# consilience-dev/llm-map-reduce-summarizer

Measured on AMD Instinct MI355X. Metric: chunks/sec (whole node) + end-to-end wall-clock, 10h transcript, Llama-3-8B, higher is better.
Workload: dtype bf16

## Files before the change

llm_map_reduce_summarizer_amd/csrc/kernels/stream_gemm.hip:

```cpp
#include "ar_common.h"

namespace {
enum { EPI_BF16 = 0, EPI_F32_PARTIAL = 1, EPI_SWIGLU = 2, EPI_SWIGLU_SPLIT = 3, EPI_RESID_SPLIT = 4 };
constexpr int SS_PARTS = 8;
constexpr int KBLK = 128;
constexpr int LDS_XTRA = 3 * 1024;
constexpr int LDS_BUDGET = 160 * 1024 - LDS_XTRA;

struct NormArgs {
    const float* ssq;
    int ssq_tiles;
    float inv_k, eps;
    bf16* resid;
    int ldr;
    float* ssp;
    int slab_m;
    mrsum_ar::TPPush tp;
};

template <int N>
__device__ __forceinline__ void wait_vmcnt() {
    static_assert(N >= 0 && N < 64, "vmcnt range");
    __builtin_amdgcn_s_waitcnt((N & 15) | (7 << 4) | (15 << 8) | ((N >> 4) << 14));
}
// ... 756 lines not shown
    }
#pragma unroll
    for (int o = 32; o > 0; o >>= 1) m = max(m, (uint32_t)__shfl_xor((int)m, o, 64));
    if ((threadIdx.x & 63) == 0) atomicMax(stats, (int)m);
}

__global__ __launch_bounds__(64) void p14_pack_kernel(const bf16* __restrict__ W, int K, unsigned char* __restrict__ P,
                                                      int* __restrict__ stats) {
    const int lane = threadIdx.x, r = lane & 15, g = lane >> 4;
    const int nkb = K / KBLK;
    const size_t tile = blockIdx.x;
    const int G = (int)(tile / nkb), kb = (int)(tile % nkb);
    const int base7 = max(stats[0] - 30, 1);
    const uint4* src = reinterpret_cast<const uint4*>(W + (size_t)(16 * G + r) * K + (size_t)kb * KBLK + 8 * g);
    uint32_t lo[8], nb[4], s2[2] = {0u, 0u};
    int bad = 0;
#pragma unroll
    for (int i = 0; i < 4; ++i) {
        const uint4 v = src[4 * i];
        const uint32_t d[4] = {v.x, v.y, v.z, v.w};
        lo[2 * i] = lo[2 * i + 1] = nb[i] = 0u;
#pragma unroll
        for (int el = 0; el < 8; ++el) {
            const uint32_t wv = (d[el >> 1] >> (16 * (el & 1))) & 0xffffu;
            const int e7 = (wv >> 8) & 0x7f, c = e7 ? e7 - base7 + 1 : 0;
            bad += e7 && (c < 1 || c > 31);
            const uint32_t c5 = (uint32_t)c & 31u, sg = wv >> 15;
            const int b = el & 3, q = 2 * (i & 1) + (el >> 2);
            lo[2 * i + (el >> 2)] |= (wv & 0xffu) << (8 * b);
            nb[i] |= (c5 & 15u) << (8 * b + 4 * (el >> 2));
            s2[i >> 1] |= (c5 >> 4) << (8 * b + 4 - q) | sg << (8 * b + 7 - (q == 3 ? 7 : q));
        }
    }
    unsigned char* t = P + tile * P14_TILE;
    *reinterpret_cast<uint4*>(t + 16 * lane) = make_uint4(lo[0], lo[1], lo[2], lo[3]);
    *reinterpret_cast<uint4*>(t + 1024 + 16 * lane) = make_uint4(lo[4], lo[5], lo[6], lo[7]);
    *reinterpret_cast<uint4*>(t + P14_NIB + 16 * lane) = make_uint4(nb[0], nb[1], nb[2], nb[3]);
    *reinterpret_cast<uint2*>(t + P14_TWO + 8 * lane) = make_uint2(s2[0], s2[1]);
    if (bad) atomicAdd(stats + 1, bad);
}
}

MRSUM_API int mrsum_p14_pack(const void* W, int N, int K, void* packed, int* stats, hipStream_t s) {
    if (N <= 0 || K <= 0 || N % 16 || K % KBLK || !W || !packed || !stats) return (int)hipErrorInvalidValue;
    hipError_t rc = hipMemsetAsync(stats, 0, 2 * sizeof(int), s);
    if (rc != hipSuccess) return (int)rc;
    const size_t n16 = (size_t)N * K / 8;
    const int blocks = (int)((n16 + 255) / 256 < 4096 ? (n16 + 255) / 256 : 4096);
    p14_max_kernel<<<blocks, 256, 0, s>>>((const uint4*)W, n16, stats);
    p14_pack_kernel<<<(unsigned)((size_t)(N / 16) * (K / KBLK)), 64, 0, s>>>((const bf16*)W, K, (unsigned char*)packed,
                                                                              stats);
    return (int)hipGetLastError();
}
```

llm_map_reduce_summarizer_amd/engine/model.py:

```python

from __future__ import annotations

import hashlib
import math
import os
from dataclasses import dataclass
from typing import Callable, List, Optional

import torch

from .. import ops
from ..ops.reference import Fp8Weight, interleave_gate_up, rope_cos_sin
from ..parallel.dist import AsyncWorks
from .config import ModelConfig


def _seed_for(seed: int, name: str) -> int:
    return int.from_bytes(hashlib.sha1(("%d:%s" % (seed, name)).encode()).digest()[:8], "little") & ((1 << 63) - 1)


def _randn(shape, std: float, seed: int, name: str, device, dtype) -> torch.Tensor:
    g = torch.Generator(device=device)
    g.manual_seed(_seed_for(seed, name))
    t = torch.randn(*shape, generator=g, device=device, dtype=torch.float32 if device.type == "cpu" else dtype)
    t.mul_(std)
    return t.to(dtype)


class _TPReduce:

    def __init__(self, model: "LlamaModel"):
        self.model = model
        ar = model.custom_ar
        self.fused = ar is not None and os.environ.get("MRSUM_FUSED_AR", "1") == "1"

    def __call__(self, t: torch.Tensor) -> torch.Tensor:
        return self.model._all_reduce(t)

    def fused_ok(self, rows: int, hidden: int) -> bool:
        ar = self.model.custom_ar
        return self.fused and ar is not None and ar.paths["fused_norm"] and rows <= ar.MAX_ROWS and \
            hidden % 4 == 0 and hidden <= 8192 and rows * hidden * 2 <= ar.max_bytes

    def add_rmsnorm(self, parts, residual, ln, eps):
        return self.model.custom_ar.add_rmsnorm(parts, residual, ln, eps)

    def push_ok(self, rows: int, hidden: int) -> bool:
        ar = self.model.custom_ar
        return ar is not None and _tp_push_enabled() and ar.push_ok(rows, hidden)

    def push_handle(self) -> int:
        return self.model.custom_ar.push_handle()

    def push_kinds(self) -> set:
        return self.model.custom_ar.push_kinds()


def _page_of(kcache: torch.Tensor, head_dim: int) -> int:
# ... 84 lines not shown
                hidden=cfg.hidden, k={"o": self.hq * self.hd, "down": self.ffn_local},
                fp8=weight_dtype == "fp8", rows=(1, 16, 64)))

    def _init_weights(self, seed: int) -> None:
        c, dev, dt = self.cfg, self.device, self.dtype
        std = c.init_std
        r, tp, hd = self.tp_rank, self.tp_size, c.head_dim
        ones = lambda: torch.ones(c.hidden, device=dev, dtype=dt)
        self.embed = _randn((c.vocab_size, c.hidden), std, seed, "embed", dev, dt)
        self.layers: List[LayerWeights] = []
        for i in range(c.n_layers):
            wq = _randn((c.n_heads * hd, c.hidden), std, seed, "l%d.wq" % i, dev, dt)
            wk = _randn((c.n_kv_heads * hd, c.hidden), std, seed, "l%d.wk" % i, dev, dt)
            wv = _randn((c.n_kv_heads * hd, c.hidden), std, seed, "l%d.wv" % i, dev, dt)
            qs, ks = self.hq * hd, self.hkv * hd
            wqkv = torch.cat([wq[r * qs:(r + 1) * qs], wk[r * ks:(r + 1) * ks], wv[r * ks:(r + 1) * ks]]).contiguous()
            del wq, wk, wv
            wo = _randn((c.hidden, c.n_heads * hd), std, seed, "l%d.wo" % i, dev, dt)
            wo = wo[:, r * qs:(r + 1) * qs].contiguous()
            f = self.ffn_local
            wg = _randn((c.ffn, c.hidden), std, seed, "l%d.wg" % i, dev, dt)
            wu = _randn((c.ffn, c.hidden), std, seed, "l%d.wu" % i, dev, dt)
            wgu = interleave_gate_up(wg[r * f:(r + 1) * f], wu[r * f:(r + 1) * f]).contiguous()
            del wg, wu
            wd = _randn((c.hidden, c.ffn), std, seed, "l%d.wd" % i, dev, dt)
            wd = wd[:, r * f:(r + 1) * f].contiguous()
            if self.weight_dtype == "fp8":
                wqkv, wo, wgu, wd = (Fp8Weight.quantize(t) for t in (wqkv, wo, wgu, wd))
            self.layers.append(LayerWeights(ones(), wqkv, wo, ones(), wgu, wd))
        self.final_norm = ones()
        lm = _randn((c.vocab_size, c.hidden), std, seed, "lm_head", dev, dt)
        v = self.vocab_local
        self.lm_head = lm[r * v:(r + 1) * v].contiguous()
        del lm
        self._quantize_lm_head()

    def _quantize_lm_head(self) -> None:
        if self.weight_dtype == "fp8" and not isinstance(self.lm_head, Fp8Weight):
            self.lm_head = Fp8Weight.quantize(self.lm_head)

    def _pack_p14(self) -> None:
        self.p14 = []
        if self.weight_dtype != "bf16" or self.tp_size != 1 or self.device.type != "cuda" \
                or self.dtype != torch.bfloat16:
            return
        hip = _hip()
        if not hip.p14_enabled():
            return
        todo = [(self.lm_head, "lm_head")]
        for lw in self.layers:
            todo += [(lw.wqkv, "qkv"), (lw.wo, "o"), (lw.wgu, "gate_up"), (lw.wdown, "down")]
        for w, role in todo:
            if hip.p14_role_used(role) and w.shape[0] % 16 == 0 and w.shape[1] % 128 == 0:
                self.p14.append(hip.p14_attach(w, role))

    def __del__(self):
        try:
            for pw in getattr(self, "p14", ()):
                _hip().p14_detach(pw.w)
        except Exception:
            pass

    def weight_bytes(self) -> int:
        def nb(t):
            return t.nbytes() if isinstance(t, Fp8Weight) else t.numel() * t.element_size()
        n = nb(self.embed) + nb(self.lm_head) + nb(self.final_norm) + sum(pw.nbytes() for pw in self.p14)
        for lw in self.layers:
            n += sum(nb(t) for t in (lw.ln1, lw.wqkv, lw.wo, lw.ln2, lw.wgu, lw.wdown))
        return n

    def local_push(self):
        if self._local_push is None:
            from ..parallel.custom_ar import LocalPush
            self._local_push = LocalPush()
        return self._local_push

    def _all_reduce(self, t: torch.Tensor) -> torch.Tensor:
        if self.tp_size > 1:
            if self.custom_ar is not None and self.custom_ar.fits(t):
                self.custom_ar.all_reduce(t)
            else:
                if t.is_cuda and torch.cuda.is_current_stream_capturing():
                    raise RuntimeError("TP all-reduce of %s does not fit the P2P buffers inside a hipGraph "
                                       "capture (lower the decode batch or raise max_bytes)" % (tuple(t.shape),))
                torch.distributed.all_reduce(t, group=self.tp_group)
        return t

    def _all_reduce_async(self, t: torch.Tensor):
        if self.tp_size == 1:
            return None
        if self.custom_ar is not None and self.custom_ar.fits(t):
            self.custom_ar.all_reduce(t)
            return None
        return torch.distributed.all_reduce(t, group=self.tp_group, async_op=True)

    def _sp_backend_ok(self) -> bool:
        return True

    def _sp_host(self) -> bool:
        return self.device.type == "cuda" and torch.distributed.get_backend(self.tp_group) != "nccl"

    def _sp_rows(self, T: int):
        Tp = -(-T // self.tp_size) * self.tp_size
        return Tp, Tp // self.tp_size

    def _sp_shard(self, t: torch.Tensor) -> torch.Tensor:
        T = t.shape[0]
# ... 203 lines not shown
```

llm_map_reduce_summarizer_amd/ops/hip.py:

```python

from __future__ import annotations

import ctypes
import os
from typing import Optional

import torch

from ._lib import kernels_lib
from .reference import Fp8Weight

_c_int, _c_float, _vp = ctypes.c_int, ctypes.c_float, ctypes.c_void_p

_SIGS = {
    "mrsum_rmsnorm": [_vp, _vp, _vp, _c_int, _c_int, _c_int, _c_int, _c_float, _vp],
    "mrsum_add_rmsnorm": [_vp, _vp, _vp, _vp, _c_int, _c_int, _c_int, _c_int, _c_float, _vp],
    "mrsum_rmsnorm_fp8": [_vp, _vp, _vp, _vp, _vp, _c_int, _c_int, _c_int, _c_int, _c_float, _c_int, _vp],
    "mrsum_rope_kv": [_vp, _c_int, _c_int, _vp, _vp, _vp, _c_int, _vp, _vp, _vp, _c_int, _c_int, _c_int, _c_int,
                      _c_int, _c_int, _vp],
    "mrsum_rope_kv_parts": [_vp, _c_int, _vp, _c_int, _c_int, _vp, _vp, _vp, _c_int, _vp, _vp, _vp, _c_int,
                            _c_int, _c_int, _c_int, _c_int, _vp],
    "mrsum_swiglu": [_vp, _vp, _c_int, _c_int, _vp],
    "mrsum_kv_scatter": [_vp, _c_int, _c_int, _c_int, _vp, _vp, _vp, _vp, _c_int, _vp],
    "mrsum_embed": [_vp, _vp, _vp, _c_int, _c_int, _c_int, _vp],
    "mrsum_attn_prefill": [_vp, _c_int, _vp, _vp, _c_int, _c_int, _vp, _c_int, _c_int, _c_int, _c_int, _c_float, _vp],
    "mrsum_attn_prefill_paged": [_vp, _c_int, _vp, _vp, _c_int, _c_int, _vp, _c_int, _c_int, _c_int, _c_int, _c_float,
                                 _vp,
                                 _vp, _vp, _c_int, _vp, _vp, _c_int, _vp],
    "mrsum_attn_decode_mfma": [_vp, _c_int, _vp, _vp, _vp, _c_int, _vp, _vp, _vp, _vp, _c_int, _c_int, _c_int,
                               _c_int, _c_int, _c_int, _c_int, _c_float, _vp, _c_int, _vp],
    "mrsum_attn_decode_rope": [_vp, _c_int, _vp, _vp, _vp, _vp, _c_int, _vp, _vp, _vp, _vp, _c_int, _c_int,
                               _c_int, _c_int, _c_int, _c_int, _c_int, _c_float, _vp, _c_int, _vp],
    "mrsum_skinny_gemm": [_vp, _c_int, _vp, _c_int, _c_int, _c_int, _vp, _c_int, _c_int, _c_int, _c_int, _vp, _c_int,
                          _c_float, _vp, _c_int, _vp, _vp, _c_int, _vp],
    "mrsum_skinny_resid_capacity_w": [_c_int],
    "mrsum_skinny_lds": [_vp, _c_int, _vp, _c_int, _c_int, _c_int, _vp, _c_int, _c_int, _c_int, _c_int, _vp],
    "mrsum_stream_gemm": [_vp, _c_int, _vp, _c_int, _c_int, _c_int, _vp, _c_int, _c_int, _c_int, _c_int, _vp, _vp,
                          _vp, _c_int, _c_float, _vp, _c_int, _vp, _c_int, _vp, _vp],
    "mrsum_stream_fp8": [_vp, _c_int, _vp, _vp, _c_int, _c_int, _c_int, _vp, _c_int, _c_int, _c_int, _c_int, _vp, _vp,
                         _vp, _c_int, _c_float, _vp, _c_int, _vp, _vp, _vp],
    "mrsum_stream_p14": [_vp, _c_int, _vp, _c_int, _c_int, _c_int, _c_int, _vp, _c_int, _c_int, _c_int, _c_int, _vp,
                         _vp, _vp, _c_int, _c_float, _vp, _c_int, _vp, _vp, _vp],
    "mrsum_p14_pack": [_vp, _c_int, _c_int, _vp, _vp, _vp],
    "mrsum_skinny_fp8": [_vp, _c_int, _vp, _vp, _c_int, _c_int, _c_int, _vp, _c_int, _c_int, _c_int, _c_int, _vp,
                         _c_int, _c_float, _vp, _c_int, _vp, _vp, _c_int, _vp],
    "mrsum_skinny_fp8_resid_capacity": [],
    "mrsum_quant_fp8_rows": [_vp, _c_int, _vp, _vp, _c_int, _c_int, _vp],
    "mrsum_add_rmsnorm_parts": [_vp, _c_int, _vp, _vp, _vp, _c_int, _c_int, _c_int, _c_float, _vp],
    "mrsum_sample_keys": [_vp, _c_int, _c_int, _c_int, _c_int, _vp, _vp, _vp, _vp, _vp],
    "mrsum_sample_finish": [_vp, _vp, _vp, _vp, _vp, _vp, _c_int, _vp, _vp, _c_int, _vp],
    "mrsum_gemm": [_vp, _c_int, _vp, _c_int, _vp, _c_int, _c_int, _c_int, _c_int, _c_int, _c_int, _vp, _vp, _c_int,
                   _c_int, _vp],
    "mrsum_sample": [_vp, _c_int, _c_int, _c_int, _vp, _vp, _vp, _vp, _vp, _vp, _vp, _vp, _vp, _c_int, _vp, _vp,
                     _vp],
    "mrsum_penalize": [_vp, _c_int, _c_int, _c_int, _c_int, _vp, _c_int, _vp, _vp, _vp, _vp, _vp, _vp],
    "mrsum_penalize_scan": [_vp, _c_int, _c_int, _c_int, _c_int, _vp, _c_int, _vp, _vp, _vp, _vp, _vp, _vp],
    "mrsum_constrain": [_vp, _c_int, _c_int, _c_int, _c_int, _vp, _vp, _c_int, _vp, _vp, _vp, _vp, _vp, _vp, _vp],
    "mrsum_sample_finish_stops": [_vp, _vp, _vp, _vp, _vp, _vp, _c_int, _vp, _vp, _vp, _c_int, _vp],
    "mrsum_sample_keys_filtered": [_vp, _c_int, _c_int, _c_int, _vp, _vp, _vp, _vp, _vp, _vp, _vp, _vp, _vp, _vp],
    "mrsum_sample_thresh": [_vp, _c_int, _c_int, _c_int, _vp, _vp, _vp, _vp, _vp, _vp, _vp],
    "mrsum_sample_filtered": [_vp, _c_int, _c_int, _c_int, _vp, _vp, _vp, _vp, _vp, _vp, _vp, _vp, _vp, _vp, _vp,
                              _vp, _vp, _c_int, _vp, _vp, _vp],
}

_fns = {}


def _fn(name: str):
    f = _fns.get(name)
    if f is None:
        lib = kernels_lib()
        f = getattr(lib, name)
        f.argtypes = _SIGS[name]
        f.restype = ctypes.c_int
        _fns[name] = f
    return f


def _stream() -> int:
    return torch.cuda.current_stream().cuda_stream


def _p(t: Optional[torch.Tensor]) -> Optional[int]:
    return None if t is None else t.data_ptr()


DEBUG_SYNC = os.environ.get("MRSUM_DEBUG_SYNC", "0") == "1"


def _check(rc: int, name: str) -> None:
    if rc != 0:
        raise RuntimeError("%s launch failed: hipError %d" % (name, rc))
    if DEBUG_SYNC and not torch.cuda.is_current_stream_capturing():
        try:
            torch.cuda.synchronize()
        except RuntimeError as e:
# ... 709 lines not shown
    N = w.shape[0]
    if M > SKINNY_MAX_M and epi in (EPI_BF16, EPI_F32_PARTIAL, EPI_SWIGLU) and norm is None:
        ch = STREAM_TALL_M
        for r0 in range(0, M, ch):
            r1 = min(M, r0 + ch)
            if r1 - r0 > SKINNY_MAX_M:
                tw = tall_wpb(N, r1 - r0, splits)
                if tw is not None:
                    o = out[:, r0:r1] if epi == EPI_F32_PARTIAL else out[r0:r1]
                    _stream_launch(x[r0:r1], w, o, epi, splits, ldo, tw, None, None, None, None, None,
                                   M if epi == EPI_F32_PARTIAL else 0)
                    continue
            for c0 in range(r0, r1, SKINNY_MAX_M):
                c1 = min(r1, c0 + SKINNY_MAX_M)
                o = out[:, c0:c1] if epi == EPI_F32_PARTIAL else out[c0:c1]
                _stream_launch(x[c0:c1], w, o, epi, splits, ldo, wpb, None, None, None, None, None,
                               M if epi == EPI_F32_PARTIAL else 0)
        return out
    return _stream_launch(x, w, out, epi, splits, ldo, wpb, parts, counters, norm, resid, ssp, 0, ar)


STREAM_TALL_M = 128
_TALL_WPB = {6: (4, 5, 6), 8: (4, 5)}


def tall_wpb(N: int, M: int, splits: int) -> Optional[int]:
    mt = 6 if M <= 96 else 8
    best, key = None, None
    for wpb in _TALL_WPB[mt]:
        if N % (16 * wpb):
            continue
        grid = N // (16 * wpb) * splits
        k = (round(grid / (-(-grid // N_CU) * N_CU), 3), wpb)
        if key is None or k > key:
            best, key = wpb, k
    return best


def _stream_launch(x, w, out, epi, splits, ldo, wpb, parts, counters, norm, resid, ssp, slab_m, ar=None):
    M, K = x.shape
    N = w.shape[0]
    _req(w.is_contiguous() and w.shape[1] == K, "stream_gemm: weight must be [N, K] contiguous")
    tall_ok = M <= 128 and epi in (EPI_BF16, EPI_F32_PARTIAL, EPI_SWIGLU) and norm is None
    _req(1 <= M and (M <= SKINNY_MAX_M or tall_ok) and K % 128 == 0 and 4 <= wpb <= 8 and N % (16 * wpb) == 0
         and (K // 128) % splits == 0, "stream_gemm: unsupported shape M=%d N=%d K=%d S=%d wpb=%d"
         % (M, N, K, splits, wpb))
    if epi in (EPI_SWIGLU_SPLIT, EPI_RESID_SPLIT):
        _req(parts is not None and parts.shape == (splits, M, N) and parts.dtype == torch.float32
             and counters is not None and counters.numel() >= N // (16 * wpb), "stream_gemm: split-K scratch")
    if epi == EPI_RESID_SPLIT:
        _req(ssp.shape[1] == N // (16 * wpb), "stream_gemm: ssp tiles")
    sq, tiles, eps = _norm_args(x, norm)
    rp, ldr, sp = _resid_args(x, N, epi, resid, ssp)
    pw = p14_lookup(w) if _P14 else None
    if pw is not None and M <= SKINNY_MAX_M and not slab_m and ar is None and p14_takes(pw.role, M):
        STATS["stream_p14"] += 1
        _check(_fn("mrsum_stream_p14")(_p(x), x.stride(0), _p(pw.packed), pw.base7, N, K, M, _p(out), ldo, epi, splits,
                                       wpb, _p(parts), _p(counters), sq, tiles, eps, rp, ldr, sp, None, _stream()),
               "stream_p14")
        return out
    STATS["stream_bf16"] += 1
    _check(_fn("mrsum_stream_gemm")(_p(x), x.stride(0), _p(w), N, K, M, _p(out), ldo, epi, splits, wpb, _p(parts),
                                    _p(counters), sq, tiles, eps, rp, ldr, sp, slab_m, ar, _stream()), "stream_gemm")
    return out


P14_ROLES = ("qkv", "o", "gate_up", "down", "lm_head")
_P14_PLAN = {("gate_up", 1), ("gate_up", 16), ("gate_up", 64), ("lm_head", 1), ("lm_head", 16),
             ("down", 1), ("down", 16)}
_P14 = {}


class PackedWeight:

    def __init__(self, w: torch.Tensor, packed: Optional[torch.Tensor], base7: int, packable: bool, role: str):
        self.w, self.packed, self.base7, self.packable, self.role = w, packed, base7, packable, role

    def nbytes(self) -> int:
        return self.packed.numel() if self.packed is not None else 0


def p14_enabled() -> bool:
    return os.environ.get("MRSUM_P14", P14_DEFAULT) == "1"


P14_DEFAULT = "1"


def p14_bucket(M: int) -> int:
    return 1 if M == 1 else 16 if M <= 16 else 64


def p14_role_used(role: str) -> bool:
    return any(r == role for r, _ in _P14_PLAN)


def p14_takes(role: str, M: int) -> bool:
    return p14_enabled() and (role, p14_bucket(M)) in _P14_PLAN


def p14_pack(w: torch.Tensor):
    _bf16_cuda(w)
    _req(w.dim() == 2 and w.is_contiguous() and w.shape[0] % 16 == 0 and w.shape[1] % 128 == 0,
         "p14_pack: expected a contiguous bf16 [16 n, 128 k] matrix")
    N, K = w.shape
    packed = torch.empty(N * K // 4 * 7, dtype=torch.uint8, device=w.device)
    stats = torch.zeros(2, dtype=torch.int32, device=w.device)
    _check(_fn("mrsum_p14_pack")(_p(w), N, K, _p(packed), _p(stats), _stream()), "p14_pack")
    mx, bad = (int(v) for v in stats.tolist())
    return packed, max(mx - 30, 1), bad


def p14_attach(w: torch.Tensor, role: str) -> PackedWeight:
    _req(role in P14_ROLES, "p14_attach: unknown role %r" % (role,))
    packed, base7, bad = p14_pack(w)
    if bad:
        print("p14: %s weight %s has %d elements outside the exponent window: bf16 kernel kept"
              % (role, tuple(w.shape), bad))
        return PackedWeight(w, None, base7, False, role)
    pw = _P14[(w.data_ptr(), w.shape[0], w.shape[1])] = PackedWeight(w, packed, base7, True, role)
    return pw


def p14_detach(w: torch.Tensor) -> None:
    _P14.pop((w.data_ptr(), w.shape[0], w.shape[1]), None)


def p14_lookup(w: torch.Tensor) -> Optional[PackedWeight]:
    return _P14.get((w.data_ptr(), w.shape[0], w.shape[1]))


def linear_takes_norm(M: int, N: int, K: int) -> bool:
    return 1 <= M <= SKINNY_MAX_M and K % 128 == 0 and stream_config(N, K, splits=1) is not None


def linear(x: torch.Tensor, w: torch.Tensor, out: Optional[torch.Tensor] = None, norm=None) -> torch.Tensor:
    M, K = x.shape
    N = w.shape[0]
    _req(norm is None or linear_takes_norm(M, N, K), "linear: a deferred norm needs a stream-GEMM shape")
    tall = (SKINNY_MAX_M < M <= STREAM_TALL_M and K % 128 == 0 and norm is None
            and stream_config(N, K, splits=1) is not None and tall_wpb(N, M, 1) is not None)
    if (M > SKINNY_MAX_M and not tall) or M == 0 or K % 128:
        return gemm(x, w, out=out)
    if out is None:
        out = torch.empty(M, N, dtype=x.dtype, device=x.device)
    _req(out.is_contiguous() and out.shape == (M, N), "linear: bad out")
    if tall:
        return _stream_gemm(x, w, out, EPI_BF16, 1, N, tall_wpb(N, M, 1))
    cfg = stream_config(N, K, splits=1)
    if cfg is not None:
        return _stream_gemm(x, w, out, EPI_BF16, 1, N, cfg[0], norm=norm)
    nt = 2 if N % 32 == 0 and N >= 16384 else 1
    if N % (16 * nt):
        return gemm(x, w, out=out)
    return _skinny(x, w, out, EPI_BF16, nt, 1, N)


def linear_parts(x: torch.Tensor, w: torch.Tensor, splits: Optional[int] = None,
                 out: Optional[torch.Tensor] = None, nt: int = 1, kernel: str = "skinny", norm=None) -> torch.Tensor:
    M, K = x.shape
    N = w.shape[0]
    if splits is None:
        splits = choose_splits(N, K, nt if kernel == "skinny" else 4)
    if out is None:
        out = torch.empty(splits, M, N, dtype=torch.float32, device=x.device)
    _req(out.is_contiguous() and out.shape == (splits, M, N) and out.dtype == torch.float32, "linear_parts: bad out")
    if kernel == "stream":
        return _stream_gemm(x, w, out, EPI_F32_PARTIAL, splits, N, nt, norm=norm)
    _req(norm is None, "linear_parts: a deferred norm needs the stream kernel")
    if kernel == "lds":
        return _skinny_lds(x, w, out, EPI_F32_PARTIAL, splits, N)
    return _skinny(x, w, out, EPI_F32_PARTIAL, nt, splits, N)


_TILE_COUNTERS = {}


def _tile_counters(device, n: int) -> torch.Tensor:
    key = (str(device), n)
    t = _TILE_COUNTERS.get(key)
    if t is None:
        _req(not torch.cuda.is_current_stream_capturing(), "split-K SwiGLU tickets first used inside a capture")
# ... 53 lines not shown
        STATS["tp_push"] += 1
    if fp8:
        _skinny_fp8(x, w, None, EPI_SKINNY_RESID, 1, 1, 0, resid=residual, ssp=ssp, ar=tp)
    else:
        _skinny(x, w, None, EPI_SKINNY_RESID, 1, 1, 0, resid=residual, ssp=ssp, ar=tp)
    return ssp


def skinny_fp8_resid_capacity() -> int:
    if "fp8" not in _RESID_CAP:
        _RESID_CAP["fp8"] = int(_fn("mrsum_skinny_fp8_resid_capacity")())
    return _RESID_CAP["fp8"]


def linear_swiglu(x: torch.Tensor, w_gu: torch.Tensor, out: Optional[torch.Tensor] = None,
                  kernel: str = "skinny", wpb: int = 4, splits: int = 1, norm=None) -> torch.Tensor:
    M = x.shape[0]
    F2 = w_gu.shape[0]
    _req(norm is None or kernel in ("stream", "stream_split", "skinny"),
         "linear_swiglu: a deferred norm needs the stream or register-streaming kernel")
    if kernel == "gemm" or M > (STREAM_MAX_M_SWIGLU if kernel == "stream" else SKINNY_MAX_M):
        return gemm(x, w_gu, out=out, swiglu=True)
    if out is None:
        out = torch.empty(M, F2 // 2, dtype=x.dtype, device=x.device)
    _req(out.is_contiguous() and out.shape == (M, F2 // 2), "linear_swiglu: bad out")
    if kernel == "stream":
        return _stream_gemm(x, w_gu, out, EPI_SWIGLU, 1, F2 // 2, wpb, norm=norm)
    if kernel == "stream_split":
        return stream_swiglu_split(x, w_gu, out, wpb, splits, norm=norm)
    if kernel == "lds":
        return _skinny_lds(x, w_gu, out, EPI_SWIGLU, 1, F2 // 2)
    return _skinny(x, w_gu, out, EPI_SWIGLU, 1, 1, F2 // 2, norm=norm)


def add_rmsnorm_parts(parts: torch.Tensor, residual: torch.Tensor, w: torch.Tensor, eps: float,
                      out: Optional[torch.Tensor] = None) -> torch.Tensor:
    _req(parts.is_cuda and parts.dtype == torch.float32 and parts.is_contiguous() and parts.dim() == 3,
         "add_rmsnorm_parts: parts must be fp32 [S, T, D]")
    _bf16_cuda(residual, w)
    S, T, D = parts.shape
    _req(residual.shape == (T, D) and residual.is_contiguous() and w.numel() == D and w.is_contiguous()
         and D % 8 == 0 and D <= 16384, "add_rmsnorm_parts: shapes")
    if out is None:
        out = torch.empty(T, D, dtype=residual.dtype, device=residual.device)
    _bf16_cuda(out)
    _rows_ok(out)
    _req(out.shape == (T, D), "add_rmsnorm_parts: bad out shape")
    _check(_fn("mrsum_add_rmsnorm_parts")(_p(parts), S, _p(residual), _p(w), _p(out), T, D, out.stride(0), eps,
                                          _stream()), "add_rmsnorm_parts")
    return out


N_CU = 256
STATS = {"tp_push": 0, "stream_p14": 0, "stream_bf16": 0}


def stream_config(N: int, K: int, swiglu: bool = False, splits: Optional[int] = None, max_splits: int = 16):
    if K % 128:
        return None
    nkb = K // 128
    best, best_key = None, None
    for wpb in (4, 5, 6, 7, 8):
        if N % (16 * wpb):
            continue
        tiles = N // (16 * wpb)
        cands = [1] if swiglu else ([splits] if splits else range(1, max_splits + 1))
        for S in cands:
            if nkb % S:
                continue
            grid = tiles * S
            eff = grid / (-(-grid // N_CU) * N_CU)
            key = (round(eff, 3), -S, wpb if grid <= 2 * N_CU else -wpb)
            if best_key is None or key > best_key:
                best, best_key = (wpb, S), key
    if best is None or best_key[0] < 0.7:
        return None
    return best


def tp_resid_config(N: int, K: int):
    best, best_key = None, None
    for wpb in (4, 8):
        if N % (16 * wpb) or (N // (16 * wpb)) % 32:
            continue
        tiles = N // (16 * wpb)
        for S in range(1, 17):
            if (K // 128) % S:
                continue
            grid = tiles * S
            eff = grid / (-(-grid // N_CU) * N_CU)
            key = (round(eff, 3), -S, wpb)
            if best_key is None or key > best_key:
                best, best_key = (wpb, S), key
    return best


def swiglu_split_config(N: int, K: int):
    best, best_key = None, None
    for wpb in (4, 7, 8):
        if N % (16 * wpb):
            continue
        tiles = N // (16 * wpb)
        for S in (1, 2, 4, 8, 16):
            if (K // 128) % S or tiles * S > 2 * N_CU:
                continue
            grid = tiles * S
            key = (round(grid / (-(-grid // N_CU) * N_CU), 3), -S, wpb)
# ... 217 lines not shown
```

llm_map_reduce_summarizer_amd/ops/reference.py:

```python

from __future__ import annotations

import math
from typing import Optional

import torch

LOG2E = 1.4426950408889634


def rmsnorm(x: torch.Tensor, w: torch.Tensor, eps: float, out: Optional[torch.Tensor] = None) -> torch.Tensor:
    xf = x.float()
    y = xf * torch.rsqrt(xf.pow(2).mean(-1, keepdim=True) + eps) * w.float()
    y = y.to(x.dtype)
    if out is not None:
        out.copy_(y)
        return out
    return y


def add_rmsnorm(x: torch.Tensor, residual: torch.Tensor, w: torch.Tensor, eps: float,
                out: Optional[torch.Tensor] = None) -> torch.Tensor:
    residual.copy_((x.float() + residual.float()).to(residual.dtype))
    return rmsnorm(residual, w, eps, out)
# ... 169 lines not shown
def p14_bits(w: torch.Tensor) -> torch.Tensor:
    return w.contiguous().view(torch.int16).to(torch.int64) & 0xffff


def p14_base7(w: torch.Tensor) -> int:
    return max(int(((p14_bits(w) >> 8) & 0x7f).max()) - (P14_WINDOW - 1), 1)


def _p14_lanes(u: torch.Tensor) -> torch.Tensor:
    N, K = u.shape
    t = u.reshape(N // 16, 16, K // 128, 4, 4, 8)
    return t.permute(0, 2, 4, 1, 3, 5).reshape(-1, 64, 4, 8)


def p14_pack_ref(w: torch.Tensor):
    N, K = w.shape
    assert w.dtype == torch.bfloat16 and N % 16 == 0 and K % 128 == 0
    u = _p14_lanes(p14_bits(w))
    base7 = p14_base7(w)
    e7 = (u >> 8) & 0x7f
    c = torch.where(e7 == 0, e7, e7 - base7 + 1)
    bad = int(((e7 != 0) & ((c < 1) | (c > P14_WINDOW))).sum())
    c5, sg = c & 31, u >> 15
    T = u.shape[0]
    lo = (u & 0xff).reshape(T, 64, 2, 16).permute(0, 2, 1, 3).reshape(T, 2048)
    q4 = c5 & 15
    nib = (q4[..., :4] | q4[..., 4:] << 4).reshape(T, 1024)
    two = torch.zeros(T, 64, 2, dtype=torch.int64, device=u.device)
    for i in range(4):
        for e in range(8):
            b, q = e & 3, 2 * (i & 1) + (e >> 2)
            two[:, :, i >> 1] |= (c5[:, :, i, e] >> 4) << (8 * b + 4 - q)
            two[:, :, i >> 1] |= sg[:, :, i, e] << (8 * b + 7 - _P14_SIGN_SHIFT[q])
    two = torch.stack([(two >> (8 * k)) & 0xff for k in range(4)], dim=-1).reshape(T, 512)
    return torch.cat([lo, nib, two], dim=1).to(torch.uint8).reshape(-1), base7, bad


def p14_unpack_ref(packed: torch.Tensor, base7: int, N: int, K: int) -> torch.Tensor:
    t = packed.reshape(-1, P14_TILE).to(torch.int64)
    T = t.shape[0]
    lo = t[:, :2048].reshape(T, 2, 64, 2, 8).permute(0, 2, 1, 3, 4).reshape(T, 64, 4, 8)
    nb = t[:, 2048:3072].reshape(T, 64, 4, 4)
    q4 = torch.cat([nb & 15, nb >> 4], dim=-1)
    tb = t[:, 3072:].reshape(T, 64, 2, 4)
    two = sum(tb[..., k] << (8 * k) for k in range(4))
    hi = torch.zeros_like(lo)
    for i in range(4):
        for e in range(8):
            b, q = e & 3, 2 * (i & 1) + (e >> 2)
            s = two[:, :, i >> 1]
            c5 = q4[:, :, i, e] | ((s >> (8 * b + 4 - q)) & 1) << 4
            e7 = torch.where(c5 == 0, c5, c5 + base7 - 1)
            hi[:, :, i, e] = ((s >> (8 * b + 7 - _P14_SIGN_SHIFT[q])) & 1) << 7 | e7
    u = (hi << 8 | lo).reshape(N // 16, K // 128, 4, 16, 4, 8).permute(0, 3, 1, 4, 2, 5).reshape(N, K)
    u = torch.where(u >= 0x8000, u - 0x10000, u)
    return u.to(torch.int16).view(torch.bfloat16)


def linear(x: torch.Tensor, w) -> torch.Tensor:
    if isinstance(w, Fp8Weight):
        return (x.float() @ w.dequant().t()).to(x.dtype)
    return torch.nn.functional.linear(x, w)


def linear_parts(x: torch.Tensor, w: torch.Tensor, splits: int = 1) -> torch.Tensor:
    K = x.shape[1]
    ks = K // splits
    wf = w.dequant() if isinstance(w, Fp8Weight) else w.float()
    return torch.stack([x[:, i * ks:(i + 1) * ks].float() @ wf[:, i * ks:(i + 1) * ks].t()
                        for i in range(splits)])


def linear_swiglu(x: torch.Tensor, w_gu) -> torch.Tensor:
    return swiglu(linear(x, w_gu))


def add_rmsnorm_parts(parts: torch.Tensor, residual: torch.Tensor, w: torch.Tensor, eps: float,
                      out: Optional[torch.Tensor] = None) -> torch.Tensor:
    residual.copy_((parts.float().sum(0) + residual.float()).to(residual.dtype))
    return rmsnorm(residual, w, eps, out)


def embed(ids: torch.Tensor, table: torch.Tensor, out: Optional[torch.Tensor] = None) -> torch.Tensor:
    y = table[ids.long().clamp(0, table.shape[0] - 1)]
    if out is not None:
        out.copy_(y)
        return out
    return y


def attn_prefill(qkv: torch.Tensor, cu_seqlens: torch.Tensor, hq: int, hkv: int, d: int, scale: float,
                 out: Optional[torch.Tensor] = None) -> torch.Tensor:
    T = qkv.shape[0]
    if out is None:
        out = torch.empty(T, hq * d, dtype=qkv.dtype, device=qkv.device)
    cu = cu_seqlens.tolist()
    g = hq // hkv
    for i in range(len(cu) - 1):
        s, e = cu[i], cu[i + 1]
        if e <= s:
            continue
        n = e - s
        q = qkv[s:e, : hq * d].view(n, hq, d).float().transpose(0, 1)
        k = qkv[s:e, hq * d: (hq + hkv) * d].view(n, hkv, d).float().transpose(0, 1)
        v = qkv[s:e, (hq + hkv) * d: (hq + 2 * hkv) * d].view(n, hkv, d).float().transpose(0, 1)
        k = k.repeat_interleave(g, dim=0)
# ... 221 lines not shown
```

Baseline: 2.258.

## Add lossless 13-bit packed weight format for gate_up decode GEMM

After: 2.280, median of 6. About the same (+1.0%).

```diff
diff --git a/llm_map_reduce_summarizer_amd/csrc/kernels/stream_gemm.hip b/llm_map_reduce_summarizer_amd/csrc/kernels/stream_gemm.hip
--- a/llm_map_reduce_summarizer_amd/csrc/kernels/stream_gemm.hip
+++ b/llm_map_reduce_summarizer_amd/csrc/kernels/stream_gemm.hip
@@ -832,3 +832,251 @@
                                                                               stats);
     return (int)hipGetLastError();
 }
+
+namespace {
+constexpr int P13_TILE = 3328, P13_NIB = 2048, P13_SGN = 3072;
+
+template <int J>
+__device__ __forceinline__ uint32_t p13_hi4(uint32_t q4, uint32_t s, uint32_t base4, uint32_t exc4) {
+    const uint32_t nz = (q4 + 0x0f0f0f0fu) & 0x10101010u;
+    const uint32_t on = (nz << 4) - (nz >> 4);
+    return ((on & (q4 + base4)) | (~on & exc4)) | ((s << J) & 0x80808080u);
+}
+
+template <int I>
+__device__ __forceinline__ bf16x8 p13_frag(uint32_t l0, uint32_t l1, uint32_t nb, uint32_t s, uint32_t base4,
+                                           uint32_t exc4) {
+    const uint32_t h0 = p13_hi4<2 * I>(nb & 0x0f0f0f0fu, s, base4, exc4);
+    const uint32_t h1 = p13_hi4<2 * I + 1>((nb >> 4) & 0x0f0f0f0fu, s, base4, exc4);
+    const u32x4 o = {__builtin_amdgcn_perm(h0, l0, 0x05010400u), __builtin_amdgcn_perm(h0, l0, 0x07030602u),
+                     __builtin_amdgcn_perm(h1, l1, 0x05010400u), __builtin_amdgcn_perm(h1, l1, 0x07030602u)};
+    return __builtin_bit_cast(bf16x8, o);
+}
+}
+
+template <int MT, int EPI, int WPB>
+__global__ __launch_bounds__(64 * WPB, 1) void stream_p13_kernel(const bf16* __restrict__ x, int ldx,
+                                                                 const unsigned char* __restrict__ W,
+                                                                 const uint32_t* __restrict__ tab, int K, int M,
+                                                                 void* __restrict__ out, int ldo, int kper,
+                                                                 float* __restrict__ parts,
+                                                                 int* __restrict__ counters, const NormArgs e) {
+    constexpr int R = 16 * WPB, BM = 16 * MT;
+    constexpr int WBYTES = WPB * P13_TILE, SLOT = WBYTES + BM * 256;
+    constexpr int D = (LDS_BUDGET / SLOT) < 8 ? (LDS_BUDGET / SLOT) : 8;
+    static_assert(D >= 2, "ring too shallow");
+    constexpr int XP = 2 * BM / 8;
+    constexpr int XI = (XP + WPB - 1) / WPB;
+    constexpr int NI = 4 + XI;
+    static_assert(NI * (D - 2) < 64, "vmcnt range");
+    __shared__ __attribute__((aligned(1024))) char lds[D * SLOT + LDS_XTRA];
+    float* const s_ss = reinterpret_cast<float*>(lds + D * SLOT + 1024);
+
+    const int tid = threadIdx.x, lane = tid & 63, w = tid >> 6;
+    const int n0 = blockIdx.x * R;
+    const int ks = blockIdx.y * kper;
+    const int nkb = kper / KBLK;
+
+    const int G = n0 / 16 + __builtin_amdgcn_readfirstlane(w);
+    const uint32_t pair = tab[G >> 1] >> (16 * (G & 1));
+    const unsigned char* const wsrc = W + ((size_t)G * (K / KBLK) + ks / KBLK) * P13_TILE;
+    const int prow = lane >> 3, pslot = lane & 7;
+    const bf16* xsrc[XI];
+    int xdst[XI];
+#pragma unroll
+    for (int i = 0; i < XI; ++i) {
+        const int q = w + WPB * i;
+        const int qq = q < XP ? q : 0;
+        const int row = 8 * (qq >> 1) + prow;
+        xsrc[i] = x + (size_t)min(row, M - 1) * ldx + ks + 8 * (8 * (qq & 1) + (pslot ^ prow));
+        xdst[i] = q < XP ? WBYTES + q * 1024 : -1;
+    }
+#define ISSUE13(slot, kb)                                                                            \
+    {                                                                                                \
+        char* base = lds + (slot) * SLOT;                                                            \
+        char* wb = base + w * P13_TILE;                                                              \
+        const unsigned char* ws = wsrc + (size_t)(kb) * P13_TILE;                                    \
+        glds16<2>(ws + 16 * lane, wb);                                                               \
+        glds16<2>(ws + 1024 + 16 * lane, wb + 1024);                                                 \
+        glds16<2>(ws + P13_NIB + 16 * lane, wb + P13_NIB);                                           \
+        glds4<2>(ws + P13_SGN + 4 * lane, wb + P13_SGN);                                             \
+        _Pragma("unroll") for (int i = 0; i < XI; ++i)                                               \
+            glds16(xsrc[i] + (kb) * KBLK, xdst[i] >= 0 ? base + xdst[i] : lds + D * SLOT);           \
+    }
+
+    f32x4 acc[MT];
+#pragma unroll
+    for (int m = 0; m < MT; ++m) acc[m] = f32x4{0.f, 0.f, 0.f, 0.f};
+
+#pragma unroll
+    for (int s = 0; s < D - 1; ++s) ISSUE13(s, min(s, nkb - 1));
+
+    const uint32_t base4 = ((pair & 0xffu) - 1u) * 0x01010101u;
+    const uint32_t exc4 = ((pair >> 8) & 0xffu) * 0x01010101u;
+    const int r = lane & 15, g = lane >> 4;
+    for (int j = 0; j < nkb; ++j) {
+        if (j + D - 2 < nkb) wait_vmcnt<NI * (D - 2)>();
+        else wait_vmcnt<0>();
+        raw_barrier();
+        if (j + D - 1 < nkb) ISSUE13((j + D - 1) % D, j + D - 1);
+        const char* wl = lds + (j % D) * SLOT + w * P13_TILE;
+        const char* xl = lds + (j % D) * SLOT + WBYTES;
+        const u32x4 lo0 = *reinterpret_cast<const u32x4*>(wl + 16 * lane);
+        const u32x4 lo1 = *reinterpret_cast<const u32x4*>(wl + 1024 + 16 * lane);
+        const u32x4 nb = *reinterpret_cast<const u32x4*>(wl + P13_NIB + 16 * lane);
+        const uint32_t sg = *reinterpret_cast<const uint32_t*>(wl + P13_SGN + 4 * lane);
+        bf16x8 av[4];
+        av[0] = p13_frag<0>(lo0[0], lo0[1], nb[0], sg, base4, exc4);
+        av[1] = p13_frag<1>(lo0[2], lo0[3], nb[1], sg, base4, exc4);
+        av[2] = p13_frag<2>(lo1[0], lo1[1], nb[2], sg, base4, exc4);
+        av[3] = p13_frag<3>(lo1[2], lo1[3], nb[3], sg, base4, exc4);
+#pragma unroll
+        for (int i = 0; i < 4; ++i) {
+#pragma unroll
+            for (int m = 0; m < MT; ++m) {
+                const u32x4 bv = *reinterpret_cast<const u32x4*>(xl + img_off(16 * m + r, 4 * i + g));
+                acc[m] = __builtin_amdgcn_mfma_f32_16x16x32_bf16(av[i], __builtin_bit_cast(bf16x8, bv), acc[m], 0, 0, 0);
+            }
+        }
+    }
+#undef ISSUE13
+
+    stream_epilogue<MT, EPI, WPB>(acc, lds, s_ss, n0, M, out, ldo, parts, counters, e);
+}
+
+MRSUM_API int mrsum_stream_p13(const void* x, int ldx, const void* W, const void* tab, int N, int K, int M, void* out,
+                               int ldo, int epi, int splits, int wpb, void* parts, int* counters, const float* ssq,
+                               int ssq_tiles, float eps, void* resid, int ldr, float* ssp, void* ar, hipStream_t s) {
+    if (M <= 0) return 0;
+    if (wpb < 4 || wpb > 8 || M > 64 || K % KBLK || N % (16 * wpb) || splits < 1 || (K / KBLK) % splits ||
+        epi < EPI_BF16 || epi > EPI_RESID_SPLIT || !tab || ((uintptr_t)tab & 3) || ar)
+        return (int)hipErrorInvalidValue;
+    const bool split_epi = epi == EPI_SWIGLU_SPLIT || epi == EPI_RESID_SPLIT;
+    if (epi != EPI_F32_PARTIAL && !split_epi && splits != 1) return (int)hipErrorInvalidValue;
+    if (split_epi && (!parts || !counters)) return (int)hipErrorInvalidValue;
+    if (epi == EPI_RESID_SPLIT && (!resid || !ssp || ldr % 4)) return (int)hipErrorInvalidValue;
+    if (ssq && (ssq_tiles <= 0 || ssq_tiles % (4 * SS_PARTS))) return (int)hipErrorInvalidValue;
+    NormArgs e;
+    e.ssq = ssq; e.ssq_tiles = ssq_tiles; e.inv_k = 1.f / (float)K; e.eps = eps;
+    e.resid = (bf16*)resid; e.ldr = ldr; e.ssp = ssp; e.slab_m = 0;
+    e.tp = mrsum_ar::tp_push_of(nullptr);
+    const int kper = K / splits;
+    const int mt = (M + 15) / 16;
+    dim3 grid(N / (16 * wpb), splits), block(64 * wpb);
+    auto X = (const bf16*)x;
+    auto Wp = (const unsigned char*)W;
+    auto T = (const uint32_t*)tab;
+    auto P = (float*)parts;
+#define L13(MT_, EPI_, WPB_) \
+    stream_p13_kernel<MT_, EPI_, WPB_><<<grid, block, 0, s>>>(X, ldx, Wp, T, K, M, out, ldo, kper, P, counters, e)
+#define BY_WPB13(MT_, EPI_)                         \
+    switch (wpb) {                                  \
+        case 4: L13(MT_, EPI_, 4); break;           \
+        case 5: L13(MT_, EPI_, 5); break;           \
+        case 6: L13(MT_, EPI_, 6); break;           \
+        case 7: L13(MT_, EPI_, 7); break;           \
+        default: L13(MT_, EPI_, 8); break;          \
+    }
+#define BY_EPI13(MT_)                                                      \
+    if (epi == EPI_BF16) { BY_WPB13(MT_, EPI_BF16) }                       \
+    else if (epi == EPI_F32_PARTIAL) { BY_WPB13(MT_, EPI_F32_PARTIAL) }    \
+    else if (epi == EPI_SWIGLU) { BY_WPB13(MT_, EPI_SWIGLU) }              \
+    else if (epi == EPI_SWIGLU_SPLIT) { BY_WPB13(MT_, EPI_SWIGLU_SPLIT) }  \
+    else { BY_WPB13(MT_, EPI_RESID_SPLIT) }
+    switch (mt) {
+        case 1: BY_EPI13(1); break;
+        case 2: BY_EPI13(2); break;
+        case 3: BY_EPI13(3); break;
+        default: BY_EPI13(4); break;
+    }
+#undef BY_EPI13
+#undef BY_WPB13
+#undef L13
+    return (int)hipGetLastError();
+}
+
+namespace {
+__global__ __launch_bounds__(256) void p13_group_kernel(const bf16* __restrict__ W, int K, unsigned char* __restrict__ tab,
+                                                        int* __restrict__ stats) {
+    __shared__ uint32_t s_set[4][4];
+    const int G = blockIdx.x, tid = threadIdx.x;
+    const uint4* src = reinterpret_cast<const uint4*>(W + (size_t)16 * G * K);
+    uint32_t set[4] = {0u, 0u, 0u, 0u};
+    for (int i = tid; i < 2 * K; i += 256) {
+        const uint4 v = src[i];
+        const uint32_t d[4] = {v.x, v.y, v.z, v.w};
+#pragma unroll
+        for (int c = 0; c < 4; ++c) {
+#pragma unroll
+            for (int h = 0; h < 2; ++h) {
+                const uint32_t e7 = (d[c] >> (8 + 16 * h)) & 0x7fu;
+#pragma unroll
+                for (int q = 0; q < 4; ++q) set[q] |= (e7 >> 5) == (uint32_t)q ? 1u << (e7 & 31u) : 0u;
+            }
+        }
+    }
+#pragma unroll
+    for (int q = 0; q < 4; ++q) {
+#pragma unroll
+        for (int o = 32; o > 0; o >>= 1) set[q] |= (uint32_t)__shfl_xor((int)set[q], o, 64);
+        if ((tid & 63) == 0) s_set[tid >> 6][q] = set[q];
+    }
+    __syncthreads();
+    if (tid == 0) {
+        int mx = 0, below = 0, exc = 0;
+        for (int v = 0; v < 128; ++v)
+            if ((s_set[0][v >> 5] | s_set[1][v >> 5] | s_set[2][v >> 5] | s_set[3][v >> 5]) >> (v & 31) & 1u) mx = v;
+        const int base7 = max(mx - 14, 1);
+        for (int v = 0; v < base7; ++v)
+            if ((s_set[0][v >> 5] | s_set[1][v >> 5] | s_set[2][v >> 5] | s_set[3][v >> 5]) >> (v & 31) & 1u) {
+                ++below;
+                exc = v;
+            }
+        tab[2 * G] = (unsigned char)base7;
+        tab[2 * G + 1] = (unsigned char)(below == 1 ? exc : 0);
+        if (below > 1) atomicAdd(stats, 1);
+    }
+}
+
+__global__ __launch_bounds__(64) void p13_pack_kernel(const bf16* __restrict__ W, int K, unsigned char* __restrict__ P,
+                                                      const unsigned char* __restrict__ tab) {
+    const int lane = threadIdx.x, r = lane & 15, g = lane >> 4;
+    const int nkb = K / KBLK;
+    const size_t tile = blockIdx.x;
+    const int G = (int)(tile / nkb), kb = (int)(tile % nkb);
+    const int base7 = tab[2 * G];
+    const uint4* src = reinterpret_cast<const uint4*>(W + (size_t)(16 * G + r) * K + (size_t)kb * KBLK + 8 * g);
+    uint32_t lo[8], nb[4], sg = 0u;
+#pragma unroll
+    for (int i = 0; i < 4; ++i) {
+        const uint4 v = src[4 * i];
+        const uint32_t d[4] = {v.x, v.y, v.z, v.w};
+        lo[2 * i] = lo[2 * i + 1] = nb[i] = 0u;
+#pragma unroll
+        for (int el = 0; el < 8; ++el) {
+            const uint32_t wv = (d[el >> 1] >> (16 * (el & 1))) & 0xffffu;
+            const int e7 = (wv >> 8) & 0x7f;
+            const uint32_t c4 = e7 >= base7 ? (uint32_t)(e7 - base7 + 1) : 0u;
+            const int b = el & 3, j = 2 * i + (el >> 2);
+            lo[2 * i + (el >> 2)] |= (wv & 0xffu) << (8 * b);
+            nb[i] |= c4 << (8 * b + 4 * (el >> 2));
+            sg |= (wv >> 15) << (8 * b + 7 - j);
+        }
+    }
+    unsigned char* t = P + tile * P13_TILE;
+    *reinterpret_cast<uint4*>(t + 16 * lane) = make_uint4(lo[0], lo[1], lo[2], lo[3]);
+    *reinterpret_cast<uint4*>(t + 1024 + 16 * lane) = make_uint4(lo[4], lo[5], lo[6], lo[7]);
+    *reinterpret_cast<uint4*>(t + P13_NIB + 16 * lane) = make_uint4(nb[0], nb[1], nb[2], nb[3]);
+    *reinterpret_cast<uint32_t*>(t + P13_SGN + 4 * lane) = sg;
+}
+}
+
+MRSUM_API int mrsum_p13_pack(const void* W, int N, int K, void* packed, void* tab, int* stats, hipStream_t s) {
+    if (N <= 0 || K <= 0 || N % 16 || K % KBLK || !W || !packed || !tab || !stats) return (int)hipErrorInvalidValue;
+    hipError_t rc = hipMemsetAsync(stats, 0, sizeof(int), s);
+    if (rc != hipSuccess) return (int)rc;
+    p13_group_kernel<<<N / 16, 256, 0, s>>>((const bf16*)W, K, (unsigned char*)tab, stats);
+    p13_pack_kernel<<<(unsigned)((size_t)(N / 16) * (K / KBLK)), 64, 0, s>>>((const bf16*)W, K, (unsigned char*)packed,
+                                                                              (const unsigned char*)tab);
+    return (int)hipGetLastError();
+}
diff --git a/llm_map_reduce_summarizer_amd/engine/model.py b/llm_map_reduce_summarizer_amd/engine/model.py
--- a/llm_map_reduce_summarizer_amd/engine/model.py
+++ b/llm_map_reduce_summarizer_amd/engine/model.py
@@ -4,6 +4,7 @@
 import hashlib
 import math
 import os
+import sys
 from dataclasses import dataclass
 from typing import Callable, List, Optional
 
@@ -194,7 +195,12 @@
             todo += [(lw.wqkv, "qkv"), (lw.wo, "o"), (lw.wgu, "gate_up"), (lw.wdown, "down")]
         for w, role in todo:
             if hip.p14_role_used(role) and w.shape[0] % 16 == 0 and w.shape[1] % 128 == 0:
-                self.p14.append(hip.p14_attach(w, role))
+                self.p14 += hip.p13_attach(w, role)
+        if self.p14:
+            forms = [pw.form if pw.packable else "bf16" for pw in self.p14]
+            print("packed decode weights: %d p13, %d p14, %d bf16 (unpackable), %.1f MiB held"
+                  % (forms.count("p13"), forms.count("p14"), forms.count("bf16"),
+                     sum(pw.nbytes() for pw in self.p14) / 2**20), file=sys.stderr)
 
     def __del__(self):
         try:
diff --git a/llm_map_reduce_summarizer_amd/ops/hip.py b/llm_map_reduce_summarizer_amd/ops/hip.py
--- a/llm_map_reduce_summarizer_amd/ops/hip.py
+++ b/llm_map_reduce_summarizer_amd/ops/hip.py
@@ -42,6 +42,9 @@
     "mrsum_stream_p14": [_vp, _c_int, _vp, _c_int, _c_int, _c_int, _c_int, _vp, _c_int, _c_int, _c_int, _c_int, _vp,
                          _vp, _vp, _c_int, _c_float, _vp, _c_int, _vp, _vp, _vp],
     "mrsum_p14_pack": [_vp, _c_int, _c_int, _vp, _vp, _vp],
+    "mrsum_stream_p13": [_vp, _c_int, _vp, _vp, _c_int, _c_int, _c_int, _vp, _c_int, _c_int, _c_int, _c_int, _vp,
+                         _vp, _vp, _c_int, _c_float, _vp, _c_int, _vp, _vp, _vp],
+    "mrsum_p13_pack": [_vp, _c_int, _c_int, _vp, _vp, _vp, _vp],
     "mrsum_skinny_fp8": [_vp, _c_int, _vp, _vp, _c_int, _c_int, _c_int, _vp, _c_int, _c_int, _c_int, _c_int, _vp,
                          _c_int, _c_float, _vp, _c_int, _vp, _vp, _c_int, _vp],
     "mrsum_skinny_fp8_resid_capacity": [],
@@ -857,8 +860,17 @@
         _req(ssp.shape[1] == N // (16 * wpb), "stream_gemm: ssp tiles")
     sq, tiles, eps = _norm_args(x, norm)
     rp, ldr, sp = _resid_args(x, N, epi, resid, ssp)
+    packed_ok = M <= SKINNY_MAX_M and not slab_m and ar is None
+    p3 = _P13.get((w.data_ptr(), N, K)) if _P13 and packed_ok else None
+    if p3 is not None and p13_takes(p3.role, M):
+        STATS["stream_p14"] += 1
+        STATS["stream_p13"] += 1
+        _check(_fn("mrsum_stream_p13")(_p(x), x.stride(0), _p(p3.packed), _p(p3.tab), N, K, M, _p(out), ldo, epi,
+                                       splits, wpb, _p(parts), _p(counters), sq, tiles, eps, rp, ldr, sp, None,
+                                       _stream()), "stream_p13")
+        return out
     pw = p14_lookup(w) if _P14 else None
-    if pw is not None and M <= SKINNY_MAX_M and not slab_m and ar is None and p14_takes(pw.role, M):
+    if pw is not None and packed_ok and p14_takes(pw.role, M):
         STATS["stream_p14"] += 1
         _check(_fn("mrsum_stream_p14")(_p(x), x.stride(0), _p(pw.packed), pw.base7, N, K, M, _p(out), ldo, epi, splits,
                                        wpb, _p(parts), _p(counters), sq, tiles, eps, rp, ldr, sp, None, _stream()),
@@ -878,11 +890,13 @@
 
 class PackedWeight:
 
-    def __init__(self, w: torch.Tensor, packed: Optional[torch.Tensor], base7: int, packable: bool, role: str):
+    def __init__(self, w: torch.Tensor, packed: Optional[torch.Tensor], base7: int, packable: bool, role: str,
+                 form: str = "p14", tab: Optional[torch.Tensor] = None):
         self.w, self.packed, self.base7, self.packable, self.role = w, packed, base7, packable, role
+        self.form, self.tab = form, tab
 
     def nbytes(self) -> int:
-        return self.packed.numel() if self.packed is not None else 0
+        return (self.packed.numel() if self.packed is not None else 0) + (self.tab.numel() if self.tab is not None else 0)
 
 
 def p14_enabled() -> bool:
@@ -929,10 +943,54 @@
 
 def p14_detach(w: torch.Tensor) -> None:
     _P14.pop((w.data_ptr(), w.shape[0], w.shape[1]), None)
+    _P13.pop((w.data_ptr(), w.shape[0], w.shape[1]), None)
 
 
 def p14_lookup(w: torch.Tensor) -> Optional[PackedWeight]:
     return _P14.get((w.data_ptr(), w.shape[0], w.shape[1]))
+
+
+_P13_PLAN = {("gate_up", 1), ("gate_up", 16)}
+_P13 = {}
+P13_DEFAULT = "1"
+
+
+def p13_enabled() -> bool:
+    return p14_enabled() and os.environ.get("MRSUM_P13", P13_DEFAULT) == "1"
+
+
+def p13_takes(role: str, M: int) -> bool:
+    return p13_enabled() and (role, p14_bucket(M)) in _P13_PLAN
+
+
+def p13_pack(w: torch.Tensor):
+    _bf16_cuda(w)
+    _req(w.dim() == 2 and w.is_contiguous() and w.shape[0] % 16 == 0 and w.shape[1] % 128 == 0,
+         "p13_pack: expected a contiguous bf16 [16 n, 128 k] matrix")
+    N, K = w.shape
+    packed = torch.empty(N * K // 8 * 13, dtype=torch.uint8, device=w.device)
+    tab = torch.zeros((N // 16 * 2 + 3) // 4 * 4, dtype=torch.uint8, device=w.device)
+    stats = torch.zeros(1, dtype=torch.int32, device=w.device)
+    _check(_fn("mrsum_p13_pack")(_p(w), N, K, _p(packed), _p(tab), _p(stats), _stream()), "p13_pack")
+    return packed, tab[:N // 16 * 2].view(N // 16, 2), int(stats.item())
+
+
+def p13_attach(w: torch.Tensor, role: str) -> list:
+    _req(role in P14_ROLES, "p13_attach: unknown role %r" % (role,))
+    made = []
+    got13 = False
+    if p13_enabled() and any(r == role for r, _ in _P13_PLAN):
+        packed, tab, bad = p13_pack(w)
+        if bad:
+            print("p13: %s weight %s has %d 16-row groups with more than one exponent value below the window: "
+                  "p14 tried" % (role, tuple(w.shape), bad))
+        else:
+            pw = _P13[(w.data_ptr(), w.shape[0], w.shape[1])] = PackedWeight(w, packed, 0, True, role, "p13", tab)
+            made.append(pw)
+            got13 = True
+    if any(r == role and not (got13 and (r, b) in _P13_PLAN) for r, b in _P14_PLAN):
+        made.append(p14_attach(w, role))
+    return made
 
 
 def linear_takes_norm(M: int, N: int, K: int) -> bool:
@@ -1092,7 +1150,7 @@
 
 
 N_CU = 256
-STATS = {"tp_push": 0, "stream_p14": 0, "stream_bf16": 0}
+STATS = {"tp_push": 0, "stream_p14": 0, "stream_p13": 0, "stream_bf16": 0}
 
 
 def stream_config(N: int, K: int, swiglu: bool = False, splits: Optional[int] = None, max_splits: int = 16):
diff --git a/llm_map_reduce_summarizer_amd/ops/reference.py b/llm_map_reduce_summarizer_amd/ops/reference.py
--- a/llm_map_reduce_summarizer_amd/ops/reference.py
+++ b/llm_map_reduce_summarizer_amd/ops/reference.py
@@ -245,6 +245,59 @@
             c5 = q4[:, :, i, e] | ((s >> (8 * b + 4 - q)) & 1) << 4
             e7 = torch.where(c5 == 0, c5, c5 + base7 - 1)
             hi[:, :, i, e] = ((s >> (8 * b + 7 - _P14_SIGN_SHIFT[q])) & 1) << 7 | e7
+    u = (hi << 8 | lo).reshape(N // 16, K // 128, 4, 16, 4, 8).permute(0, 3, 1, 4, 2, 5).reshape(N, K)
+    u = torch.where(u >= 0x8000, u - 0x10000, u)
+    return u.to(torch.int16).view(torch.bfloat16)
+
+
+P13_TILE = 3328
+P13_WINDOW = 15
+
+
+def p13_pack_ref(w: torch.Tensor):
+    N, K = w.shape
+    assert w.dtype == torch.bfloat16 and N % 16 == 0 and K % 128 == 0
+    bits = p14_bits(w)
+    e7g = ((bits >> 8) & 0x7f).reshape(N // 16, 16 * K)
+    base = (e7g.max(dim=1).values - (P13_WINDOW - 1)).clamp(min=1)
+    below = e7g < base[:, None]
+    lo_b = torch.where(below, e7g, torch.full_like(e7g, 127)).min(dim=1).values
+    hi_b = torch.where(below, e7g, torch.full_like(e7g, -1)).max(dim=1).values
+    some = below.any(dim=1)
+    unpackable = some & (lo_b != hi_b)
+    exc = torch.where(some & ~unpackable, lo_b, torch.zeros_like(lo_b))
+    tab = torch.stack([base, exc], dim=1).to(torch.uint8)
+    u = _p14_lanes(bits)
+    T = u.shape[0]
+    tbase = base.repeat_interleave(K // 128)[:, None, None, None]
+    e7 = (u >> 8) & 0x7f
+    c4 = torch.where(e7 >= tbase, e7 - tbase + 1, torch.zeros_like(e7))
+    sg = u >> 15
+    lo = (u & 0xff).reshape(T, 64, 2, 16).permute(0, 2, 1, 3).reshape(T, 2048)
+    nib = (c4[..., :4] | c4[..., 4:] << 4).reshape(T, 1024)
+    sd = torch.zeros(T, 64, dtype=torch.int64, device=u.device)
+    for i in range(4):
+        for e in range(8):
+            sd |= sg[:, :, i, e] << (8 * (e & 3) + 7 - (2 * i + (e >> 2)))
+    sgn = torch.stack([(sd >> (8 * k)) & 0xff for k in range(4)], dim=-1).reshape(T, 256)
+    return torch.cat([lo, nib, sgn], dim=1).to(torch.uint8).reshape(-1), tab, int(unpackable.sum())
+
+
+def p13_unpack_ref(packed: torch.Tensor, tab: torch.Tensor, N: int, K: int) -> torch.Tensor:
+    t = packed.reshape(-1, P13_TILE).to(torch.int64)
+    T = t.shape[0]
+    tab = tab.reshape(N // 16, 2).to(torch.int64).repeat_interleave(K // 128, dim=0)
+    base, exc = tab[:, 0, None, None, None], tab[:, 1, None, None, None]
+    lo = t[:, :2048].reshape(T, 2, 64, 2, 8).permute(0, 2, 1, 3, 4).reshape(T, 64, 4, 8)
+    nb = t[:, 2048:3072].reshape(T, 64, 4, 4)
+    c4 = torch.cat([nb & 15, nb >> 4], dim=-1)
+    sb = t[:, 3072:].reshape(T, 64, 4)
+    sd = sum(sb[..., k] << (8 * k) for k in range(4))
+    e7 = torch.where(c4 == 0, exc.expand_as(c4), c4 + base - 1)
+    hi = torch.zeros_like(lo)
+    for i in range(4):
+        for e in range(8):
+            hi[:, :, i, e] = ((sd >> (8 * (e & 3) + 7 - (2 * i + (e >> 2)))) & 1) << 7 | e7[:, :, i, e]
     u = (hi << 8 | lo).reshape(N // 16, K // 128, 4, 16, 4, 8).permute(0, 3, 1, 4, 2, 5).reshape(N, K)
     u = torch.where(u >= 0x8000, u - 0x10000, u)
     return u.to(torch.int16).view(torch.bfloat16)
```
